# haotianteng/Chiron

Hardware: AMD Instinct MI355X
Metric: kilobases/sec basecalled (DNA_default seg_len=400 batch=1100) (higher is better)
Workload: dtype f32; 1 GPU; DNA_default seg_len=400 jump=390 batch=1100 greedy, synthetic 4 kHz signal (BASELINE.json configs[1]); segment_len=400, jump=390, batch=1100, decode=greedy, weights=seeded synthetic (exact checkpoint shapes), parallelism=reads sharded per GPU, no collective, slots_in_flight=3, parallelism_bookkeeping=none (one rank), distinct_devices=1

## Files before the change

### chiron_amd/csrc/engine.hip

```cpp
#include <hip/hip_runtime.h>

#include <algorithm>
#include <atomic>
#include <chrono>
#include <cfloat>
#include <cmath>
#include <cstdarg>
#include <cstdio>
#include <cstring>
#include <cstdlib>
#include <map>
#include <mutex>
#include <string>
#include <vector>

#include "../../include/chiron_amd.h"
#include "kernels.h"
#include "model_layout.h"
#include "weight_pack.h"
#include <dlfcn.h>

static const char* const kProfNames[] = {"conv_dma", "lstm_proj_dma", "lstm_recurrence", "fc_head", "ctc_greedy", "ctc_beam", "sparse_build",
                                         "path_prob", "conv_lift", "conv_res", "conv1_pwl", "conv_wino", "lstm_proj0_dma", "conv2a"};

// ... 2 lines not shown
static thread_local char g_err[512] = "";
namespace chiron {
chiron_status set_error(chiron_status st, const char* fmt, ...) {
  va_list ap;
  va_start(ap, fmt);
  vsnprintf(g_err, sizeof(g_err), fmt, ap);
  va_end(ap);
  return st;
}
}
static constexpr auto& fail = chiron::set_error;
#define HIP_TRY(expr)                                                                              \
  do {                                                                                             \
    hipError_t _e = (expr);                                                                        \
    if (_e != hipSuccess)                                                                          \
      return fail(CHIRON_ERR_DEVICE, "%s failed: %s (%s:%d)", #expr, hipGetErrorString(_e), __FILE__, \
                  __LINE__);                                                                       \
  } while (0)

extern "C" const char* chiron_last_error(void) { return g_err; }
extern "C" int32_t chiron_abi_version(void) { return CHIRON_ABI_VERSION; }

static int g_timing_build = 0;
static char g_timing_source[96] = "";
namespace chiron {
void mark_timing_build(const char* source) {
  g_timing_build = 1;
  snprintf(g_timing_source, sizeof(g_timing_source), "%s", source ? source : "?");
}
}
extern "C" uint32_t chiron_build_flags(void) { return g_timing_build ? CHIRON_BUILD_TIMING : 0u; }

extern "C" chiron_status chiron_device_pci_bus_id(int32_t device_id, char* out, size_t cap) {
  if (!out || cap < 16) return chiron::set_error(CHIRON_ERR_INVALID, "chiron_device_pci_bus_id: buffer of at least 16 bytes needed");
  int n = 0;
  if (hipGetDeviceCount(&n) != hipSuccess || n <= 0) return chiron::set_error(CHIRON_ERR_DEVICE, "no HIP device");
  if (device_id < 0 || device_id >= n) return chiron::set_error(CHIRON_ERR_INVALID, "device %d of %d", device_id, n);
  hipError_t err = hipDeviceGetPCIBusId(out, (int)cap, device_id);
  if (err != hipSuccess) return chiron::set_error(CHIRON_ERR_DEVICE, "hipDeviceGetPCIBusId: %s", hipGetErrorString(err));
  for (char* c = out; *c; ++c)
    if (*c >= 'A' && *c <= 'F') *c += 'a' - 'A';
  return CHIRON_OK;
}

extern "C" chiron_status chiron_weights_size(const chiron_model_desc* d, size_t* n_floats) {
  BlobMap map;
  chiron_status st = blob_map(d, &map);
  if (st) return st;
  if (!n_floats) return fail(CHIRON_ERR_INVALID, "null n_floats");
  *n_floats = map.total;
  return CHIRON_OK;
}

#define CHIRON_LSTM_WIDE_DEFAULT 2

struct CalibRecord {
  const float* shift;
  int k0, cin;
  int lstm_layer, lstm_dir, lstm_part;
  double rows;
  size_t slot;
};
struct CalibCtx {
  double* dev_sums = nullptr;
  size_t max_records = 0;
  std::vector<CalibRecord> rec;
  int skipped = 0;
};

struct ProfEvent {
  int name_id;
  hipEvent_t a, b;
  double flops, bytes;
};

struct Slot {
  hipStream_t stream = nullptr;
  unsigned long long* tile_ctr = nullptr;
  unsigned long long tile_base = 0;
  unsigned long long tile_base32 = 0;
  float* sig = nullptr;
  int32_t* seq = nullptr;
  float* act[5] = {nullptr, nullptr, nullptr, nullptr, nullptr};
  double* bn_sums = nullptr;
  float* z = nullptr;
  float* lasth[2] = {nullptr, nullptr};
  float* lasth_f32 = nullptr;
  float* logits = nullptr;
  uint8_t* labels = nullptr;
  int32_t* count = nullptr;
  float* log_prob = nullptr;
  float* prob = nullptr;
  int64_t* offsets = nullptr;
  int64_t* indices = nullptr;
  int64_t* values = nullptr;
  int64_t* meta = nullptr;
  void* beam_ws = nullptr;
  size_t beam_ws_bytes = 0;
  float* h_sig = nullptr;
  int32_t* h_seq = nullptr;
  int64_t* h_indices = nullptr;
  int64_t* h_values = nullptr;
  int64_t* h_meta = nullptr;
  float* h_log_prob = nullptr;
  float* h_prob = nullptr;
  float* h_logits = nullptr;
  uint8_t* h_labels = nullptr;
// ... 57 lines not shown
  int calibrated = 0;
  std::vector<void*> owned;
  bool profiling = false;
  std::vector<std::string> prof_names;
  std::mutex mu;
};

static chiron_status dev_alloc(chiron_engine* e, void** p, size_t bytes, bool zero) {
  HIP_TRY(hipMalloc(p, bytes ? bytes : 16));
  e->owned.push_back(*p);
  if (zero) HIP_TRY(hipMemset(*p, 0, bytes ? bytes : 16));
  return CHIRON_OK;
}
static chiron_status upload_plans(chiron_engine* e, std::vector<Upload>& ups) {
  for (Upload& u : ups) {
    chiron_status st = dev_alloc(e, u.dst, u.bytes, false);
    if (st) return st;
    HIP_TRY(hipMemcpy(*u.dst, u.data, u.bytes, hipMemcpyHostToDevice));
    u.owner.reset();
    if (u.host.Npad > 0) e->plan_host[(const float*)*u.dst] = std::move(u.host);
  }
  return CHIRON_OK;
}

static bool split_row_scale() {
  static const bool on = getenv("CHIRON_SPLIT_NO_ROW_SCALE") == nullptr;
  return on;
}

static chiron_status build_plans(chiron_engine* e, const float* w) {
  e->bn_batch = e->desc.bn_mode == CHIRON_BN_BATCH;
  PackSwitches sw;
  sw.no_winograd = getenv("CHIRON_NO_WINOGRAD") != nullptr;
  sw.wino_f2 = getenv("CHIRON_WINOGRAD_F2") != nullptr;
  sw.wino_f4 = getenv("CHIRON_WINOGRAD_F4") != nullptr;
  sw.no_pwl = getenv("CHIRON_NO_PWL") != nullptr;
  sw.split_rec32 = getenv("CHIRON_SPLIT_REC32") != nullptr;
  if (e->split) sw.split_row_scale = split_row_scale();
  std::vector<Upload> ups;
  chiron_status st = pack_weights(e->desc, e->map, w, e->L, e->opts.dtype, sw, e, &ups);
  if (st) return st;
  if (e->proj_bf16 && e->opts.dtype == CHIRON_F32 && !e->bn_batch) {
    for (LstmPlan& lp : e->lstm) {
      ConvGemmPlan& g = lp.proj[0];
      if (lp.nproj != 1 || (lp.in_w != 256 && lp.in_w != 200) || g.N % BF3_BN != 0) continue;
      for (const Upload& u : ups) {
        if (u.dst != reinterpret_cast<void**>(&g.Wt)) continue;
        const std::vector<uint16_t> planes = bf16x3_planes(static_cast<const float*>(u.data), g.N, g.K, lp.in_w);
        if ((st = dev_alloc(e, &g.w_bf3, planes.size() * sizeof(uint16_t), false))) return st;
        HIP_TRY(hipMemcpy(g.w_bf3, planes.data(), planes.size() * sizeof(uint16_t), hipMemcpyHostToDevice));
      }
    }
  }
  return upload_plans(e, ups);
}

static const uint64_t TENSOR_LIMIT = 0xFFFE0000ull;

static chiron_status plan_sizes(const chiron_model_desc* d, const chiron_engine_opts* o, chiron_engine_sizes* out) {
  BlobMap map;
  chiron_status st = blob_map(d, &map);
  if (st) return st;
  if (!o) return fail(CHIRON_ERR_INVALID, "null opts");
  if (o->max_batch < 1 || o->segment_len < 1) return fail(CHIRON_ERR_INVALID, "max_batch/segment_len must be positive");
  if (o->dtype != CHIRON_F32 && o->dtype != CHIRON_F16 && o->dtype != CHIRON_F32_SPLIT && o->dtype != CHIRON_F16_W2)
    return fail(CHIRON_ERR_INVALID, "dtype %d unknown (0 = f32, 1 = f16, 2 = f32 as hi/lo half pairs, 3 = f16 activations against hi/lo weights)", o->dtype);
  if (o->max_beam < 0) return fail(CHIRON_ERR_INVALID, "max_beam %d", o->max_beam);
  const bool f16 = o->dtype == CHIRON_F16 || o->dtype == CHIRON_F16_W2, split = o->dtype == CHIRON_F32_SPLIT, bn_batch = d->bn_mode == CHIRON_BN_BATCH;
  const uint64_t B = (uint64_t)o->max_batch, BP = (uint64_t)roundup(o->max_batch, 16), L = (uint64_t)o->segment_len, H = d->hidden, K = d->classes;
  SiteFrames fr[MAX_SITES];
  const uint64_t T = (uint64_t)frames(map, o->segment_len, fr);
  uint64_t tmax = 0, cmax = 0;
  for (int i = map.has_stem; i < map.n_sites; ++i) {
    tmax = std::max<uint64_t>(tmax, (uint64_t)std::max(fr[i].tin, fr[i].tout));
    cmax = std::max<uint64_t>(cmax, (uint64_t)map.site[i].co);
  }
  const uint64_t lasth_ld = !split ? 2 * H : d->rnn_kind == CHIRON_RNN_MULTI ? 2 * (uint64_t)roundup(d->hidden, 32) : (uint64_t)roundup(2 * d->hidden, 32);
  const uint64_t act = B * tmax * cmax * (f16 ? 2 : 4), lasth = T * BP * lasth_ld * 4, z = T * BP * 2 * 4 * H * 4;
  if (B * tmax >= (1ull << 31) || T * BP >= (1ull << 31))
    return fail(CHIRON_ERR_OVERFLOW, "max_batch %d x %llu frames does not fit the kernels' int row index", o->max_batch, (unsigned long long)tmax);
  if (act > TENSOR_LIMIT)
    return fail(CHIRON_ERR_OVERFLOW, "max_batch %d: an activation tensor [%d x %llu x %llu] needs %llu bytes, the kernels address at most %llu "
                "per tensor (about %llu windows at this segment length and dtype): use a smaller max_batch",
                o->max_batch, o->max_batch, (unsigned long long)tmax, (unsigned long long)cmax, (unsigned long long)act,
                (unsigned long long)TENSOR_LIMIT, (unsigned long long)(TENSOR_LIMIT / (tmax * cmax * (f16 ? 2 : 4))));
  if (T * BP * lasth_ld * (f16 ? 2 : 4) > TENSOR_LIMIT)
    return fail(CHIRON_ERR_OVERFLOW, "max_batch %d: the recurrent output [%llu x %llu x %llu] needs %llu bytes, the kernels address at most %llu per tensor",
                o->max_batch, (unsigned long long)T, (unsigned long long)BP, (unsigned long long)lasth_ld, (unsigned long long)lasth,
                (unsigned long long)TENSOR_LIMIT);
  uint64_t slot = B * L * 4 + BP * 4 + (bn_batch ? 5 : 3) * act + (bn_batch ? 2 * 2 * cmax * 8 : 0) + z + 2 * lasth + (split ? T * BP * 2 * H * 4 : 0);
  slot += B * T * K * 4 + B * T + 3 * B * 4 + (B + 1) * 8 + B * T * 16 + B * T * 8 + 3 * 8;
  if (o->max_beam > 0) slot += beam_workspace_bytes((int)B, (int)T, o->max_beam);
  if (out) {
    out->T = (int32_t)T;
    out->ratio = (double)o->segment_len / (double)T;
    out->largest_tensor_bytes = std::max(act, T * BP * lasth_ld * (f16 ? 2 : 4));
    out->tensor_limit_bytes = TENSOR_LIMIT;
    out->slot_bytes = slot;
    out->total_bytes = slot * (uint64_t)std::max(1, o->n_slots);
  }
  return CHIRON_OK;
}

extern "C" chiron_status chiron_engine_plan(const chiron_model_desc* desc, const chiron_engine_opts* opts, chiron_engine_sizes* out) {
  if (!out) return fail(CHIRON_ERR_INVALID, "null out");
  memset(out, 0, sizeof(*out));
// ... 46 lines not shown
  s->h_flat = (uint8_t*)malloc(B * T ? B * T : 1);
  if (!s->h_flat) return fail(CHIRON_ERR_DEVICE, "out of host memory");
  memset(s->h_prob, 0, B * 4);
  return CHIRON_OK;
}

extern "C" chiron_status chiron_engine_create(const chiron_model_desc* desc, const float* weights, size_t n_floats,
                                              const chiron_engine_opts* opts, chiron_engine** out) {
  if (!out) return fail(CHIRON_ERR_INVALID, "null out");
  *out = nullptr;
  BlobMap map;
  chiron_status st = blob_map(desc, &map);
  if (st) return st;
  if (!weights || !opts) return fail(CHIRON_ERR_INVALID, "null weights/opts");
  if (map.total != n_floats) return fail(CHIRON_ERR_INVALID, "weight blob has %zu floats, descriptor needs %zu", n_floats, map.total);
  {
    chiron_engine_sizes sz;
    if ((st = plan_sizes(desc, opts, &sz))) return st;
  }
  if (desc->hidden != 100) return fail(CHIRON_ERR_INVALID, "hidden=%d: the recurrence kernel is built for hidden=100 (both shipped models)", desc->hidden);
  const bool trace = getenv("CHIRON_TRACE_CREATE") != nullptr;
  auto now = [] { return std::chrono::duration<double, std::milli>(std::chrono::steady_clock::now().time_since_epoch()).count(); };
  const double t_enter = now();
  int ndev = 0;
  if (hipGetDeviceCount(&ndev) != hipSuccess || ndev < 1) return fail(CHIRON_ERR_DEVICE, "no HIP device visible: libchiron_amd has no CPU fallback");
  if (opts->device_id < 0 || opts->device_id >= ndev) return fail(CHIRON_ERR_INVALID, "device_id %d out of range (%d devices)", opts->device_id, ndev);
  HIP_TRY(hipSetDevice(opts->device_id));
  if (trace) HIP_TRY(hipFree(nullptr));
  const double t_runtime = now();

  chiron_engine* e = new chiron_engine();
  e->desc = *desc;
  e->map = map;
  e->opts = *opts;
  if (e->opts.n_slots < 1) e->opts.n_slots = 1;
  e->L = opts->segment_len;
  e->H = desc->hidden;
  e->K = desc->classes;
  e->maxB = opts->max_batch;
  e->BP = roundup(opts->max_batch, 16);
  e->w2 = opts->dtype == CHIRON_F16_W2;
  e->w2_zf16 = e->w2 && getenv("CHIRON_W2_ZF16") != nullptr;
  e->lasth32 = getenv("CHIRON_F16_LASTH16") == nullptr;
  e->f16 = opts->dtype == CHIRON_F16 || e->w2;
  e->split = opts->dtype == CHIRON_F32_SPLIT;
  e->kq = e->f16 ? 2 * GEMM_BK : GEMM_BK;
  e->lasth_ld = !e->split ? 2 * desc->hidden
                : desc->rnn_kind == CHIRON_RNN_MULTI ? 2 * roundup(desc->hidden, 32) : roundup(2 * desc->hidden, 32);
  e->lstm_paired = getenv("CHIRON_LSTM_PAIR") != nullptr;
  e->lstm_fixed_roles = getenv("CHIRON_LSTM_FIXED_ROLES") != nullptr;
  {
    const char* wv = getenv("CHIRON_LSTM_WIDE");
    e->lstm_form = wv ? atoi(wv) : (e->split ? 0 : CHIRON_LSTM_WIDE_DEFAULT);
    if (e->lstm_form < 0 || e->lstm_form > 2) e->lstm_form = CHIRON_LSTM_WIDE_DEFAULT;
  }
  e->lstm16_narrow = getenv("CHIRON_LSTM16_NARROW") != nullptr;
  e->lstm16_pair = getenv("CHIRON_LSTM16_PAIR") ? atoi(getenv("CHIRON_LSTM16_PAIR")) : -1;
  e->stream16 = getenv("CHIRON_NO_STREAM16") == nullptr && opts->dtype != CHIRON_F16_W2;
  e->stream32 = getenv("CHIRON_NO_STREAM32") == nullptr;
  e->proj_bf16 = getenv("CHIRON_PROJ_FP32") == nullptr;
  e->dyn_tiles = getenv("CHIRON_STATIC_TILES") == nullptr;
  {
    const int min_groups = getenv("CHIRON_LSTM16_FUSED_MIN") ? atoi(getenv("CHIRON_LSTM16_FUSED_MIN")) : 64;
    e->lstm16_fused = e->f16 && !e->w2 && !e->lstm16_narrow && desc->hidden == 100 && (e->BP / 16) * 2 >= min_groups && getenv("CHIRON_LSTM16_UNFUSED") == nullptr;
  }
  if (e->f16 && !e->w2) e->host_weights.assign(weights, weights + n_floats);
  st = build_plans(e, weights);
  const double t_plans = now();
  if (st == CHIRON_OK) {
    e->slots.resize(e->opts.n_slots);
    for (Slot& s : e->slots)
      if ((st = alloc_slot(e, &s))) break;
  }
  const double t_slots = now();
  if (st == CHIRON_OK && hipDeviceSynchronize() != hipSuccess) st = fail(CHIRON_ERR_DEVICE, "device sync after setup failed");
  if (trace)
    fprintf(stderr, "chiron_engine_create: {\"hip_runtime_and_context_ms\": %.1f, \"weights_prepared_and_uploaded_ms\": %.1f, \"slot_buffers_ms\": %.1f, "
                    "\"final_sync_ms\": %.1f, \"slots\": %d}\n", t_runtime - t_enter, t_plans - t_runtime, t_slots - t_plans, now() - t_slots, e->opts.n_slots);
  if (st) {
    chiron_engine_destroy(e);
    return st;
  }
  e->prof_names.assign(std::begin(kProfNames), std::end(kProfNames));
  *out = e;
  return CHIRON_OK;
}

extern "C" void chiron_engine_destroy(chiron_engine* e) {
  if (!e) return;
  hipSetDevice(e->opts.device_id);
  hipDeviceSynchronize();
  for (Slot& s : e->slots) {
    for (ProfEvent& ev : s.events) {
      hipEventDestroy(ev.a);
      hipEventDestroy(ev.b);
    }
    if (s.stream) hipStreamDestroy(s.stream);
    void* sp[] = {s.score.labels, s.score.label_len, s.score.loss, s.score.edit, s.score.status, s.score.ws};
    for (void* q : sp)
      if (q) hipFree(q);
    void* hp[] = {s.h_sig, s.h_seq, s.h_indices, s.h_values, s.h_meta, s.h_log_prob, s.h_prob, s.h_logits, s.h_labels, s.h_count};
    free(s.h_flat);
    for (void* q : hp)
      if (q) hipHostFree(q);
  }
  for (void* q : e->owned) hipFree(q);
  delete e;
// ... 272 lines not shown
          Prof pr(e, s, PN_CONV, 2.0 * B * b.t_out * (double)b.k * b.c * b.c, 4.0 * B * (b.t_in + b.t_out) * b.c);
          ok &= launch(e, g, s->stream);
        }
      }
      g = gemm_desc(e, b.gc, B, Mout, b.t_out,
                    {GemmSeg{bufB, b.c, 0, b.c, cop, b.t_out, 1, 0, 0}, GemmSeg{x, b.c_in, 0, b.c_in, cip, b.t_in, b.stride, 0, 0}}, 1, bufA, b.c);
      {
        Prof pr(e, s, PN_CONV, 2.0 * B * b.t_out * (double)(b.c + b.c_in) * b.c, 4.0 * B * b.t_out * (2.0 * b.c + b.c_in));
        ok &= launch(e, g, s->stream);
      }
      x = bufA;
      xi = ia;
    }
  }
  s->sig_used = x;
  return ok;
}

static bool run_rnn(chiron_engine* e, Slot* s, int B) {
  bool ok = true;
  bool last_out_f32 = false;
  const float* fea = s->sig_used;
  const int T = e->T, H = e->H, BP = e->BP;
  const int zc = 4 * H;
  const float* prev = nullptr;
  for (size_t l = 0; l < e->lstm.size(); ++l) {
    const LstmPlan& lp = e->lstm[l];
    float* outbuf = s->lasth[l & 1];
    const bool fused = e->lstm16_fused && lp.wxwide != nullptr;
    for (int pj = 0; pj < (fused ? 0 : lp.nproj); ++pj) {
      const int Kp = roundup(lp.in_w, e->kq);
      const GemmSeg src = l == 0           ? GemmSeg{fea, e->C, 0, e->C, Kp, T, 1, 0, 0}
                          : lp.nproj == 1 ? GemmSeg{prev, e->lasth_ld, 0, 2 * H, Kp, T, 1, 0, 1}
                                          : GemmSeg{prev, e->lasth_ld, e->split ? pj * roundup(H, 32) : pj * H, H, Kp, T, 1, 0, 1};
      GemmParams g = gemm_desc(e, lp.proj[pj], B, (long)T * BP, T, {src}, 0, s->z, 0);
      g.m_time_major = 1;
      g.out_mode = 1;
      g.z_cols = zc;
      g.z_ndir = lp.nproj == 1 ? 2 : 1;
      g.z_dir0 = lp.nproj == 1 ? 0 : pj;
      g.z_seq_len = s->seq;
      g.w_bf3 = lp.proj[pj].w_bf3;
      g.z_f16 = (e->f16 && (!e->w2 || e->w2_zf16)) ? 1 : 0;
      const double ndir = lp.nproj == 1 ? 2.0 : 1.0;
      Prof pr(e, s, l == 0 ? PN_PROJ0 : PN_PROJ, 2.0 * B * T * (double)lp.in_w * 4 * H * ndir, 4.0 * B * T * (lp.in_w + ndir * zc));
      ok &= launch(e, g, s->stream);
    }
    LstmParams r;
    r.z = s->z;
    r.wfrag = lp.wfrag;
    r.wlight = lp.wlight;
    r.wwide = lp.wwide;
    r.wwide32 = lp.wwide32;
    r.wsplit = lp.wsplit;
    r.form32 = e->lstm_form;
    r.narrow16 = e->lstm16_narrow ? 1 : 0;
    r.xsrc = nullptr;
    r.wxwide = nullptr;
    r.whfused = nullptr;
    r.fused_pair = 0;
    r.xbias = nullptr;
    r.xK = r.xld = r.x_time_major = 0;
    if (fused) {
      r.xsrc = l == 0 ? (const void*)fea : (const void*)prev;
      r.wxwide = lp.wxwide;
      r.whfused = lp.whfused;
      r.fused_pair = e->lstm16_pair >= 0 ? (e->lstm16_pair ? 1 : 0) : ((BP / 16) * 2 > current_device_cus() ? 1 : 0);
      r.xbias = lp.proj[0].shift;
      r.xK = lp.in_w;
      r.xld = l == 0 ? e->C : e->lasth_ld;
      r.x_time_major = l == 0 ? 0 : 1;
    }
    r.seq_len = s->seq;
    r.out = e->split ? s->lasth_f32 : outbuf;
    r.out_f32 = (e->f16 && e->lasth32 && e->calib == nullptr && l + 1 == e->lstm.size()) ? 1 : 0;
    last_out_f32 = r.out_f32 != 0;
    const bool direct_split = e->split && lp.wsplit != nullptr && l + 1 < e->lstm.size();
    r.out_split = direct_split ? (void*)outbuf : nullptr;
    r.split_ld = e->lasth_ld;
    r.split_bw0 = e->desc.rnn_kind == CHIRON_RNN_MULTI ? roundup(H, 32) : H;
    r.T = T;
    r.B = B;
    r.BP = BP;
    r.H = H;
    r.ndir = 2;
    r.paired = e->lstm_paired ? 1 : 0;
    r.fixed_roles = e->lstm_fixed_roles ? 1 : 0;
    r.group0 = 0;
    r.f16 = e->f16 ? 1 : 0;
    r.w2 = e->w2 ? (e->w2_zf16 ? 2 : 1) : 0;
    if (e->calib && e->f16) {
      for (int pj = 0; pj < lp.nproj; ++pj) {
        const int dir = lp.nproj == 1 ? -1 : pj;
        if (l == 0)
          calib_measure(e, lp.proj[pj].shift, 0, fea, (long)B * T, e->C, 0, e->C, 0, B, (int)l, dir, 0, s->stream);
        else
          calib_measure(e, lp.proj[pj].shift, 0, prev, (long)T * BP, e->lasth_ld, lp.nproj == 1 ? 0 : pj * H, lp.in_w, BP, B, (int)l, dir, 0, s->stream);
      }
    }
    {
      Prof pr(e, s, PN_REC, 2.0 * 2.0 * B * T * (double)H * 4 * H + (fused ? 2.0 * B * T * (double)lp.in_w * 4 * H * 2.0 : 0.0),
              fused ? (e->f16 ? 2.0 : 4.0) * B * T * (2.0 * lp.in_w + 2.0 * H) : 4.0 * B * T * 2.0 * (zc + H));
      launch_lstm(r, s->stream);
    }
    if (e->calib && e->f16)
      for (int dir = 0; dir < 2; ++dir)
// ... 601 lines not shown
```

### chiron_amd/csrc/kernels.h

```cpp
#pragma once
#include <hip/hip_runtime.h>
#include <stdint.h>

#include "../../include/chiron_amd.h"

#define CHIRON_KMAX 5

namespace chiron {

constexpr int CHIRON_MAX_DEVICES = 64;
inline int current_device_index() {
  int dev = 0;
  if (hipGetDevice(&dev) != hipSuccess || dev < 0 || dev >= CHIRON_MAX_DEVICES) dev = 0;
  return dev;
}
inline int current_device_cus() {
  static int n_cu[CHIRON_MAX_DEVICES] = {};
  const int dev = current_device_index();
  int n = __atomic_load_n(&n_cu[dev], __ATOMIC_RELAXED);
  if (n == 0) {
    hipDeviceProp_t prop;
    n = hipGetDeviceProperties(&prop, dev) == hipSuccess ? prop.multiProcessorCount : 0;
    if (n <= 0) n = 256;
    __atomic_store_n(&n_cu[dev], n, __ATOMIC_RELAXED);
// ... 39 lines not shown
  const float* sig;
  int L;
  const float* lift_a;
  const float* lift_b;
  const float* res_a;
  const float* res_b;
  int res_stride;
  float* out;
  int ldo;
  int out_mode;
  int z_cols;
  int z_ndir;
  int z_dir0;
  int z_dirs_total;
  const int32_t* z_seq_len;
  int f16;
  int z_f16;
  unsigned long long* tile_ctr;
  unsigned long long tile_base;
  unsigned long long* tile_base_host;
};

bool launch_gemm(const GemmParams& p, hipStream_t stream);
bool launch_stream16(const GemmParams& p, hipStream_t stream);
bool launch_stream32(const GemmParams& p, hipStream_t stream);


struct WinoParams {
  const float* src;
  const float* U;
  const float* shift;
  float* out;
  int B, T, C, N, lda, ldo, relu;
  int f4;
  unsigned long long* tile_ctr;
  unsigned long long tile_base;
  unsigned long long* tile_base_host;
};
bool launch_wino_conv3(const WinoParams& p, hipStream_t stream);

constexpr int LSTM_K = 100;
constexpr int LSTM_NW = 7;

struct LstmParams {
  const float* z;
  const float* wfrag;
  const float* wlight;
  const float* wwide32;
  int out_f32;
  const void* wsplit;
  void* out_split;
  int split_ld;
  int split_bw0;
  int form32;
  const void* wwide;
  const void* xsrc;
  const void* wxwide;
  const void* whfused;
  int fused_pair;
  const float* xbias;
  int xK, xld, x_time_major;
  const int32_t* seq_len;
  float* out;
  int T, B, BP, H;
  int ndir;
  int paired;
  int fixed_roles;
  int group0;
  int narrow16;
  int w2;
  int f16;
};
void launch_lstm(const LstmParams& p, hipStream_t stream);
constexpr int LSTM_KSTEPS16 = 25;

void launch_stem_conv(const float* sig, const float* w, const float* shift, void* out, int B, int L, int T_out, int k, int stride, int left,
                      int C, int fmt, int relu, hipStream_t stream);
void launch_split_convert(const float* src, void* dst, long rows, int cols, int ld, int half, int half_dst, hipStream_t stream);
struct PwlConvParams {
  const float* sig;
  const float* bp;
  const float* ref;
  const float2* tab;
  const float* shift;
  void* out;
  int B, L, T_out, k, stride, left, C, nbp;
  int fmt;
};
bool launch_pwl_conv(const PwlConvParams& p, hipStream_t stream);

void launch_lift(const float* sig, const float* a, const float* b, void* out, long n_pos, int C, int fmt ,
                 hipStream_t stream);

struct FcParams {
  const float* lasth;
  const float* w;
  const float* bias;
  const float* wc;
  const float* bc;
  float* logits;
  int T, B, BP, H, K;
  int f16;
  int split;
  int ld;
};
void launch_fc(const FcParams& p, hipStream_t stream);
// ... 169 lines not shown
```

### chiron_amd/csrc/lstm.hip

```cpp
#include "kernels.h"
#include "timing_variants.h"

#include <algorithm>

#pragma clang fp contract(off)

namespace chiron {

typedef float f32x4 __attribute__((ext_vector_type(4)));

constexpr int HG = 8 * 64;

#ifndef CHIRON_GATE_MATH
#define CHIRON_GATE_MATH 0
#endif
typedef float f32x2 __attribute__((ext_vector_type(2)));
constexpr float LOG2E = 1.4426950408889634f;
#if CHIRON_GATE_MATH == 3
__device__ __forceinline__ float sym_tanh(float x) {
  const float e = __builtin_amdgcn_exp2f(__builtin_fabsf(x) * (-2.0f * LOG2E));
  const float t = (1.0f - e) * __builtin_amdgcn_rcpf(1.0f + e);
  return __builtin_copysignf(t, x);
}
#endif
// ... 1303 lines not shown
      if (partial && ch == wave) {
#pragma unroll
        for (int j = 0; j < 8; ++j) {
#pragma unroll
          for (int n = 0; n < 3; ++n) acc[n] = __builtin_amdgcn_mfma_f32_16x16x4f32(w[n][8 * ch + j], hv[ch & 1][j], (ch == 0 && j == 0) ? zero4 : acc[n], 0, 0, 0);
          accp = __builtin_amdgcn_mfma_f32_16x16x4f32(wp[j], hv[ch & 1][j], j == 0 ? zero4 : accp, 0, 0, 0);
        }
      } else {
#pragma unroll
        for (int j = 0; j < 8; ++j)
#pragma unroll
          for (int n = 0; n < 3; ++n) {
#if CHIRON_SENS & 8
            if (j & 1) { acc[n][0] += w[n][8 * ch + j] * hv[ch & 1][j]; continue; }
#endif
            acc[n] = __builtin_amdgcn_mfma_f32_16x16x4f32(w[n][8 * ch + j], hv[ch & 1][j], (ch == 0 && j == 0) ? zero4 : acc[n], 0, 0, 0);
          }
      }
      __builtin_amdgcn_sched_barrier(0);
    }
    __syncthreads();
    const float h24 = hb[(W32_KS - 1) * 64];
#pragma unroll
    for (int n = 0; n < 3; ++n) acc[n] = __builtin_amdgcn_mfma_f32_16x16x4f32(w[n][W32_KS - 1], h24, acc[n], 0, 0, 0);
    f32x4 acc24 = {0.f, 0.f, 0.f, 0.f};
    if (owner24) acc24 = __builtin_amdgcn_mfma_f32_16x16x4f32(wp[0], h24, (f32x4){0.f, 0.f, 0.f, 0.f}, 0, 0, 0);
    asm volatile("s_waitcnt vmcnt(0)" : "+v"(z4[0]), "+v"(z4[1]), "+v"(z4[2]), "+v"(z24) : : "memory");
    if (owner24) reinterpret_cast<f32x4*>(part)[192 + lane] = acc24 + z24;
    if (s > 0) flush(s - 1, cur);
    if (partial) reinterpret_cast<f32x4*>(part)[wave * 64 + lane] = accp;
#pragma unroll
    for (int n = 0; n < 3; ++n) {
      float hnew;
      c[n] = sens_cell(acc[n] + z4[n], c[n], &hnew);
      hbuf[(cur ^ 1) * HW32 + (tile0 + n) * 64 + lane] = hnew;
    }
    cur ^= 1;
    __syncthreads();
  }
  if (maxlen > 0) {
    if (owner24) finish24(cur);
    __syncthreads();
    flush(maxlen - 1, cur);
  }

  for (int s = maxlen; s < p.T; ++s)
    for (int i = tid; i < 16 * p.H; i += 64 * W16_NW) {
      const int r = i / p.H;
      const int uu = i - r * p.H;
      p.out[((long)s * p.BP + g16 * 16 + r) * outw + dir * p.H + uu] = 0.f;
    }
}

static int lstm_cu_count() { return current_device_cus(); }

void launch_lstm(const LstmParams& p0, hipStream_t stream) {
  LstmParams p = p0;
  p.group0 = 0;
  const int groups = p.BP / 4;
  if (p.f16 && p.xsrc) {
    const int g16 = p.BP / 16;
    const dim3 blk(64 * W16_NW);
    if (p.out_f32) {
      static const bool attr_ok = [] {
        return hipFuncSetAttribute(reinterpret_cast<const void*>(lstm16f_kernel<8, 2, true>), hipFuncAttributeMaxDynamicSharedMemorySize, 3 * 2 * 32 * 128 * 2 + 16) == hipSuccess &&
               hipFuncSetAttribute(reinterpret_cast<const void*>(lstm16f_kernel<7, 2, true>), hipFuncAttributeMaxDynamicSharedMemorySize, 3 * 2 * 28 * 128 * 2 + 16) == hipSuccess &&
               hipFuncSetAttribute(reinterpret_cast<const void*>(lstm16f_kernel<8, 1, true>), hipFuncAttributeMaxDynamicSharedMemorySize, 3 * 32 * 128 * 2 + 16) == hipSuccess &&
               hipFuncSetAttribute(reinterpret_cast<const void*>(lstm16f_kernel<7, 1, true>), hipFuncAttributeMaxDynamicSharedMemorySize, 3 * 28 * 128 * 2 + 16) == hipSuccess;
      }();
      (void)attr_ok;
    }
    if (g16 % 2 == 0 && p.fused_pair) {
      const dim3 grd((g16 / 2) * p.ndir);
      if (p.xK > 224) {
        if (p.out_f32) hipLaunchKernelGGL((lstm16f_kernel<8, 2, true>), grd, blk, 3 * 2 * 32 * 128 * 2 + 16, stream, p);
        else hipLaunchKernelGGL((lstm16f_kernel<8, 2>), grd, blk, 3 * 2 * 32 * 128 * 2 + 16, stream, p);
      } else {
        if (p.out_f32) hipLaunchKernelGGL((lstm16f_kernel<7, 2, true>), grd, blk, 3 * 2 * 28 * 128 * 2 + 16, stream, p);
        else hipLaunchKernelGGL((lstm16f_kernel<7, 2>), grd, blk, 3 * 2 * 28 * 128 * 2 + 16, stream, p);
      }
    } else {
      const dim3 grd(g16 * p.ndir);
      if (p.xK > 224) {
        if (p.out_f32) hipLaunchKernelGGL((lstm16f_kernel<8, 1, true>), grd, blk, 3 * 32 * 128 * 2 + 16, stream, p);
        else hipLaunchKernelGGL((lstm16f_kernel<8, 1>), grd, blk, 3 * 32 * 128 * 2 + 16, stream, p);
      } else {
        if (p.out_f32) hipLaunchKernelGGL((lstm16f_kernel<7, 1, true>), grd, blk, 3 * 28 * 128 * 2 + 16, stream, p);
        else hipLaunchKernelGGL((lstm16f_kernel<7, 1>), grd, blk, 3 * 28 * 128 * 2 + 16, stream, p);
      }
    }
    return;
  }
  if (p.f16 && p.w2) {
    if (p.w2 == 2)
      hipLaunchKernelGGL(lstm16w2_kernel<true>, dim3((p.BP / 16) * p.ndir), dim3(64 * W16_NW), 0, stream, p);
    else
      hipLaunchKernelGGL(lstm16w2_kernel<false>, dim3((p.BP / 16) * p.ndir), dim3(64 * W16_NW), 0, stream, p);
    return;
  }
  if (p.f16) {
    const int wide = (p.wwide && !p.narrow16 && (p.BP / 16) * p.ndir >= lstm_cu_count()) ? p.BP / 16 : 0;
    if (wide > 0) hipLaunchKernelGGL(lstm16w_kernel, dim3(wide * p.ndir), dim3(64 * W16_NW), 0, stream, p);
    p.group0 = 4 * wide;
    if (groups > p.group0) hipLaunchKernelGGL(lstm16_kernel, dim3((groups - p.group0) * p.ndir), dim3(64 * LSTM_NW), 0, stream, p);
    return;
  }
  if (p.wsplit) {
    hipLaunchKernelGGL(lstm32s_kernel, dim3((p.BP / 16) * p.ndir), dim3(64 * W16_NW), 0, stream, p);
    return;
  }
  if (p.wwide32 && p.form32 > 0 && !p.paired) {
    if (p.form32 == 2)
      hipLaunchKernelGGL(lstm32w2_kernel, dim3((p.BP / 16) * p.ndir), dim3(64 * W16_NW), 0, stream, p);
    else
      hipLaunchKernelGGL(lstm32w_kernel, dim3((p.BP / 16) * p.ndir), dim3(64 * W16_NW), 0, stream, p);
    return;
  }
  const int n_cu = lstm_cu_count();
  const int pairs = p.paired ? std::min(groups / 2, n_cu / p.ndir) : 0;
  if (pairs > 0) hipLaunchKernelGGL(lstm_kernel<2>, dim3(pairs * p.ndir), dim3(64 * LSTM_NW * 2), 0, stream, p);
  p.group0 = 2 * pairs;
  if (groups > p.group0) hipLaunchKernelGGL(lstm_kernel<1>, dim3((groups - p.group0) * p.ndir), dim3(64 * LSTM_NW), 0, stream, p);
}

}
```

### chiron_amd/csrc/weight_pack.h

```cpp
#pragma once
#include <algorithm>
#include <cfloat>
#include <cmath>
#include <cstdint>
#include <cstring>
#include <memory>
#include <utility>
#include <vector>

#include "kernels.h"
#include "model_layout.h"

namespace chiron {

inline int roundup(int v, int m) { return (v + m - 1) / m * m; }

struct ConvGemmPlan {
  float* Wt = nullptr;
  float* shift = nullptr;
  float* descale = nullptr;
  void* w_bf3 = nullptr;
  int N = 0, Npad = 0, K = 0;
};

struct PlanHost {
  std::vector<float> dW;
  std::vector<float> shift0;
  int N = 0, Npad = 0, K = 0;
};

struct BlockPlan {
  bool lift = false;
  int c_in = 0, c = 0, k = 0, stride = 1, left = 0;
  int t_in = 0, t_out = 0;
  float *lift_a = nullptr, *lift_b = nullptr;
  float *res_a = nullptr, *res_b = nullptr;
  float *pwl_bp = nullptr, *pwl_ref = nullptr, *pwl_tab = nullptr, *pwl_shift = nullptr;
  int pwl_nbp = 0;
  ConvGemmPlan ga, gb, gc;
  float* wino_u = nullptr;
  int wino_f4 = 0;
  ConvGemmPlan g1;
  bool i_bn = false;
  float *bn_scale[4] = {nullptr, nullptr, nullptr, nullptr}, *bn_offset[4] = {nullptr, nullptr, nullptr, nullptr};
};

struct LstmPlan {
  int in_w = 0;
  ConvGemmPlan proj[2];
  int nproj = 1;
  float* wfrag = nullptr;
  void* wwide = nullptr;
  void* whfused = nullptr;
  void* wxwide = nullptr;
  int wx_ksteps = 0;
  void* wsplit = nullptr;
  float* wwide32 = nullptr;
  float* wlight = nullptr;
};

struct NetPlans {
  int T = 0, C = 0;
  int stem_k = 0, stem_stride = 1, stem_left = 0, stem_t = 0, stem_c = 0;
  float *stem_w = nullptr, *stem_shift = nullptr, *stem_scale = nullptr, *stem_offset = nullptr;
  std::vector<BlockPlan> blocks;
  std::vector<LstmPlan> lstm;
  float *fc_w = nullptr, *fc_b = nullptr, *fc_wc = nullptr, *fc_bc = nullptr;
};

struct PackSwitches {
  bool no_winograd = false;
  bool wino_f2 = false;
  bool wino_f4 = false;
  bool no_pwl = false;
  bool split_rec32 = false;
  bool split_row_scale = true;
};

struct Upload {
  void** dst;
  std::shared_ptr<void> owner;
  const void* data;
  size_t bytes;
  PlanHost host;
};


struct HalfPair {
  _Float16 hi, lo;
};
inline HalfPair split_half(float v) {
  const _Float16 hi = (_Float16)v;
  return {hi, (_Float16)(v - (float)hi)};
}

struct Bf16x3 {
  uint16_t hi, mid, lo;
};
inline uint32_t f32_bits(float v) {
  uint32_t u;
  memcpy(&u, &v, 4);
  return u;
}
inline float bits_f32(uint32_t u) {
  float v;
  memcpy(&v, &u, 4);
  return v;
}
inline Bf16x3 split_bf16x3(float w) {
  const uint32_t hb = f32_bits(w) & 0xffff0000u;
// ... 33 lines not shown
    const float inv = (1.0f / sqrtf(var[i] + 1e-5f)) * scale[i];
    f.inv[i] = inv;
    f.sh[i] = offset[i] - mean[i] * inv;
  }
  return f;
}

inline void fold_filter(std::vector<float>& Wt, std::vector<float>& shift, int K, int k0, const float* W, int taps, int ci, int co, int cop,
                        const float* inv, const float* sh) {
  for (int n = 0; n < co; ++n) {
    for (int tap = 0; tap < taps; ++tap)
      for (int c = 0; c < ci; ++c) {
        const float v = W[((size_t)tap * ci + c) * co + n];
        Wt[(size_t)n * K + k0 + tap * cop + c] = inv ? v * inv[n] : v;
      }
    if (sh) shift[n] = k0 == 0 ? sh[n] : shift[n] + sh[n];
  }
}

struct LstmKernels {
  const float* kern[2];
  int H;
  float at(int dir, int k_off, int width, int k, int g, int unit) const {
    return k < width && unit < H ? kern[dir][(size_t)(k_off + k) * 4 * H + g * H + unit] : 0.f;
  }
};

template <class Put>
inline void narrow_fragments(const LstmKernels& kn, int V, int ksteps, int k_off, int width, Put put) {
  for (int dir = 0; dir < 2; ++dir)
    for (int wv = 0; wv < LSTM_NW; ++wv)
      for (int ks = 0; ks < ksteps; ++ks)
        for (int lane = 0; lane < 64; ++lane)
          for (int q = 0; q < V; ++q) {
            const int k = V * ks + q, g = lane >> 4, unit = 16 * wv + (lane & 15);
            put(((((size_t)dir * LSTM_NW + wv) * ksteps + ks) * 64 + lane) * V + q, kn.at(dir, k_off, width, k, g, unit));
          }
}
inline size_t narrow_elems(int V, int ksteps) { return (size_t)2 * LSTM_NW * ksteps * 64 * V; }

template <class Put>
inline void wide_fragments(const LstmKernels& kn, int V, int ksteps, int k_off, int width, Put put) {
  for (int dir = 0; dir < 2; ++dir)
    for (int wv = 0; wv < 8; ++wv)
      for (int slot = 0; slot < (wv == 7 ? 4 : 3); ++slot)
        for (int ks = 0; ks < ksteps; ++ks)
          for (int lane = 0; lane < 64; ++lane)
            for (int q = 0; q < V; ++q) {
              const int k = V * (4 * ks + (lane >> 4)) + q, g = lane & 3, unit = 4 * (3 * wv + slot) + ((lane >> 2) & 3);
              put((((((size_t)dir * 8 + wv) * 4 + slot) * ksteps + ks) * 64 + lane) * V + q, kn.at(dir, k_off, width, k, g, unit));
            }
}
inline size_t wide_elems(int V, int ksteps) { return (size_t)2 * 8 * 4 * ksteps * 64 * V; }

inline std::vector<float> light_fragment(const LstmKernels& kn, int k_off) {
  std::vector<float> wl((size_t)2 * 28 * 64, 0.f);
  for (int dir = 0; dir < 2; ++dir)
    for (int m = 0; m < 28; ++m)
      for (int lane = 0; lane < 64; ++lane) {
        const int q = m >> 2, a = m & 3, kg = lane >> 4, g = (lane >> 2) & 3, j = lane & 3;
        const int k = 16 * q + 4 * kg + a;
        wl[((size_t)dir * 28 + m) * 64 + lane] = kn.at(dir, k_off, kn.H, k, g, 96 + j);
      }
  return wl;
}

struct WeightPacker {
  const chiron_model_desc& d;
  const BlobMap& map;
  const float* w;
  const PackSwitches sw;
  const bool f16, w2, split, batch;
  const int kq;
  NetPlans* out;
  std::vector<Upload>* ups;

  template <class P, class Tp>
  Upload& put(P** dst, std::vector<Tp>&& h) {
    auto v = std::make_shared<std::vector<Tp>>(std::move(h));
    ups->push_back(Upload{reinterpret_cast<void**>(dst), v, v->data(), v->size() * sizeof(Tp), PlanHost()});
    return ups->back();
  }

  void gemm(ConvGemmPlan* g, std::vector<float>&& Wt, std::vector<float>&& shift, int N, int Npad, int K) {
    g->N = N;
    g->Npad = Npad;
    g->K = K;
    if (split) {
      std::vector<_Float16> h(2 * Wt.size());
      std::vector<float> sh2(std::move(shift)), ds((size_t)Npad + 192, 1.0f);
      for (int n = 0; n < Npad; ++n) {
        float mx = 0.f;
        for (int k = 0; k < K; ++k) mx = std::max(mx, fabsf(Wt[(size_t)n * K + k]));
        int s = 0;
        if (sw.split_row_scale && mx > 0.f && std::isfinite(mx)) {
          int ex;
          frexpf(mx, &ex);
          s = std::min(60, std::max(-60, 13 - ex));
          if (n < (int)sh2.size() && !std::isfinite(ldexpf(sh2[n], s))) s = 0;
        }
        ds[n] = ldexpf(1.0f, -s);
        if (n < (int)sh2.size()) sh2[n] = ldexpf(sh2[n], s);
        for (int k = 0; k < K; ++k) {
          const size_t i = (size_t)n * K + k;
          const HalfPair p = split_half(ldexpf(Wt[i], s));
          const size_t blk = i / 32, el = i % 32;
// ... 295 lines not shown
```

Measured before the change: 5010 kbases/s.

## Run f32 LSTM recurrence as bf16x3 split MFMA by default

Adds a new LSTM recurrence kernel (form 3, now the default) that splits the recurrent weights and hidden state into three bf16 planes each. The first 96 of the K dimension is accumulated with nine 16x16x32 bf16 MFMA cross terms, and the remaining slice uses an f32 MFMA. The hidden state is re-split into bf16 planes in LDS at every step. The aim is to replace slow f32 4-wide MFMA work in the serial recurrence with denser bf16 MFMA while keeping near-f32 accuracy, at the cost of more MFMA instructions, more registers and extra LDS traffic.

```diff
diff --git a/chiron_amd/csrc/engine.hip b/chiron_amd/csrc/engine.hip
--- a/chiron_amd/csrc/engine.hip
+++ b/chiron_amd/csrc/engine.hip
@@ -78,7 +78,7 @@
   return CHIRON_OK;
 }
 
-#define CHIRON_LSTM_WIDE_DEFAULT 2
+#define CHIRON_LSTM_WIDE_DEFAULT 3
 
 struct CalibRecord {
   const float* shift;
@@ -242,6 +242,13 @@
       }
     }
   }
+  for (LstmPlan& lp : e->lstm)
+    for (const Upload& u : ups) {
+      if (u.dst != reinterpret_cast<void**>(&lp.wwide32)) continue;
+      const std::vector<uint16_t> frag = rec_bf16x3_fragments(static_cast<const float*>(u.data));
+      if ((st = dev_alloc(e, &lp.wrec_bf3, frag.size() * sizeof(uint16_t), false))) return st;
+      HIP_TRY(hipMemcpy(lp.wrec_bf3, frag.data(), frag.size() * sizeof(uint16_t), hipMemcpyHostToDevice));
+    }
   return upload_plans(e, ups);
 }
 
@@ -394,7 +401,7 @@
   {
     const char* wv = getenv("CHIRON_LSTM_WIDE");
     e->lstm_form = wv ? atoi(wv) : (e->split ? 0 : CHIRON_LSTM_WIDE_DEFAULT);
-    if (e->lstm_form < 0 || e->lstm_form > 2) e->lstm_form = CHIRON_LSTM_WIDE_DEFAULT;
+    if (e->lstm_form < 0 || e->lstm_form > 3) e->lstm_form = CHIRON_LSTM_WIDE_DEFAULT;
   }
   e->lstm16_narrow = getenv("CHIRON_LSTM16_NARROW") != nullptr;
   e->lstm16_pair = getenv("CHIRON_LSTM16_PAIR") ? atoi(getenv("CHIRON_LSTM16_PAIR")) : -1;
@@ -773,6 +780,7 @@
     r.wlight = lp.wlight;
     r.wwide = lp.wwide;
     r.wwide32 = lp.wwide32;
+    r.wrec_bf3 = lp.wrec_bf3;
     r.wsplit = lp.wsplit;
     r.form32 = e->lstm_form;
     r.narrow16 = e->lstm16_narrow ? 1 : 0;
diff --git a/chiron_amd/csrc/kernels.h b/chiron_amd/csrc/kernels.h
--- a/chiron_amd/csrc/kernels.h
+++ b/chiron_amd/csrc/kernels.h
@@ -115,6 +115,7 @@
   void* out_split;
   int split_ld;
   int split_bw0;
+  const void* wrec_bf3;
   int form32;
   const void* wwide;
   const void* xsrc;
diff --git a/chiron_amd/csrc/lstm.hip b/chiron_amd/csrc/lstm.hip
--- a/chiron_amd/csrc/lstm.hip
+++ b/chiron_amd/csrc/lstm.hip
@@ -1379,6 +1379,187 @@
     }
 }
 
+typedef __bf16 bf16x8 __attribute__((ext_vector_type(8)));
+constexpr int REC_BF3_TERMS = 9;
+constexpr bool REC_BF3_SMALL_FIRST = true;
+constexpr bool REC_BF3_LEAN = false;
+constexpr int HPL = 3 * 3 * 64;
+
+template <bool LEAN>
+__global__ __launch_bounds__(64 * W16_NW, 1) void lstm32w2_kernel_bf3(const LstmParams p) {
+  __shared__ __attribute__((aligned(16))) float hbuf[2 * HW32];
+  __shared__ __attribute__((aligned(16))) float part[4 * 256];
+  __shared__ __attribute__((aligned(16))) f32x4 hpl[2 * HPL];
+  __shared__ __attribute__((aligned(16))) f32x4 wp_lds[LEAN ? 3 * 3 * 64 : 1];
+
+  const int tid = threadIdx.x;
+  const int lane = tid & 63;
+  const int wave = __builtin_amdgcn_readfirstlane(tid >> 6);
+  const int dir = blockIdx.x % p.ndir;
+  const int g16 = blockIdx.x / p.ndir;
+  const int tile0 = 3 * wave;
+  const bool partial = wave < 3, owner24 = wave == W16_NW - 1;
+  const f32x4 zero4 = {0.f, 0.f, 0.f, 0.f};
+
+  bf16x8 wb[3][3][3], wpb[3];
+  float wl[3], wp0 = 0.f;
+  {
+    const f32x4* wrec = reinterpret_cast<const f32x4*>(p.wrec_bf3) + (long)dir * 25 * 9 * 64 + lane;
+#pragma unroll
+    for (int n = 0; n < 3; ++n)
+#pragma unroll
+      for (int j = 0; j < 9; ++j) wb[n][j / 3][j % 3] = __builtin_bit_cast(bf16x8, wrec[((tile0 + n) * 9 + j) * 64]);
+    const float* wf = p.wwide32 + ((long)dir * W16_NW + wave) * W16_NT * W32_KS * 64 + lane;
+#pragma unroll
+    for (int n = 0; n < 3; ++n) wl[n] = wf[(n * W32_KS + W32_KS - 1) * 64];
+    if (owner24) wp0 = p.wwide32[((((long)dir * W16_NW + 7) * W16_NT + 3) * W32_KS + W32_KS - 1) * 64 + lane];
+#pragma unroll
+    for (int pl = 0; pl < 3; ++pl) {
+      f32x4 v = zero4;
+      if (partial) v = wrec[((24 * 3 + wave) * 3 + pl) * 64];
+      if (LEAN) {
+        if (partial) wp_lds[(wave * 3 + pl) * 64 + lane] = v;
+      } else {
+        wpb[pl] = __builtin_bit_cast(bf16x8, v);
+      }
+    }
+  }
+  for (int i = tid; i < 2 * HW32; i += 64 * W16_NW) hbuf[i] = 0.f;
+  for (int i = tid; i < 2 * HPL; i += 64 * W16_NW) hpl[i] = zero4;
+
+  const int row = lane & 15, q = lane >> 4;
+  int maxlen = 0;
+#pragma unroll
+  for (int r = 0; r < 16; ++r) maxlen = max(maxlen, min(p.seq_len[g16 * 16 + r], p.T));
+  __syncthreads();
+
+  const unsigned outw = p.ndir * p.H;
+  const unsigned zcols = 4 * p.H;
+  const unsigned zstep = (p.BP >> 2) * p.ndir * zcols * 4;
+  const unsigned zlo = (((((g16 * 4 + (row >> 2)) * p.ndir + dir) * zcols + 4 * tile0 + q) * 4) + (row & 3)) * 4;
+  const unsigned zhi = zlo + 2 * 1600;
+  const unsigned ostep = p.BP * outw;
+  const int hpw = row * 8 + q;
+
+  const int f_len = min(p.seq_len[g16 * 16 + (lane & 15)], p.T);
+  auto flush = [&](int sp, int buf) {
+    int lo = lane;
+    asm volatile("" : "+v"(lo));
+    const int fr = lo & 15, fq = 4 * wave + (lo >> 4);
+    if (fq < 25) {
+      const bool act = sp < f_len;
+      const unsigned to = (dir == 0 || !act) ? sp : f_len - 1 - sp;
+      const float* hp = hbuf + buf * HW32 + fq * 64 + fr;
+      f32x4 v = {hp[0], hp[16], hp[32], hp[48]};
+      if (!act) v = zero4;
+      *reinterpret_cast<f32x4*>(p.out + (to * ostep + (g16 * 16 + fr) * outw + dir * p.H + 4 * fq)) = v;
+    }
+  };
+
+  float c[3] = {0.f, 0.f, 0.f};
+  float c24 = 0.f;
+  int cur = 0;
+
+  auto finish24 = [&](int buf) {
+    const f32x4* pp = reinterpret_cast<const f32x4*>(part) + lane;
+    f32x4 sum = pp[0] + pp[64];
+    sum = sum + pp[128];
+    float hnew;
+    c24 = sens_cell(sum + pp[192], c24, &hnew);
+    hbuf[buf * HW32 + 24 * 64 + lane] = hnew;
+  };
+
+  constexpr int TERMS[9][2] = {{2, 2}, {2, 1}, {1, 2}, {2, 0}, {1, 1}, {0, 2}, {1, 0}, {0, 1}, {0, 0}};
+  constexpr int T0 = 9 - REC_BF3_TERMS;
+
+  for (int s = 0; s < maxlen; ++s) {
+    const float* zs = p.z + (size_t)s * zstep;
+    f32x4 z4[3], z24 = zero4;
+    W32_ZLOAD(z4[0][0], zlo, 0);   W32_ZLOAD(z4[0][1], zlo, 1600);   W32_ZLOAD(z4[0][2], zhi, 0);   W32_ZLOAD(z4[0][3], zhi, 1600);
+    W32_ZLOAD(z4[1][0], zlo, 64);  W32_ZLOAD(z4[1][1], zlo, 1664);   W32_ZLOAD(z4[1][2], zhi, 64);  W32_ZLOAD(z4[1][3], zhi, 1664);
+    W32_ZLOAD(z4[2][0], zlo, 128); W32_ZLOAD(z4[2][1], zlo, 1728);   W32_ZLOAD(z4[2][2], zhi, 128); W32_ZLOAD(z4[2][3], zhi, 1728);
+    if (owner24) {
+      W32_ZLOAD(z24[0], zlo, 192); W32_ZLOAD(z24[1], zlo, 1792); W32_ZLOAD(z24[2], zhi, 192); W32_ZLOAD(z24[3], zhi, 1792);
+    }
+    if (owner24 && s > 0) finish24(cur);
+    const f32x4* hp = hpl + cur * HPL + lane;
+    f32x4 acc[3], accp = zero4;
+    bf16x8 hb[LEAN ? 2 : 3][3];
+#pragma unroll
+    for (int j = 0; j < (LEAN ? 3 : 9); ++j) hb[LEAN ? 0 : j % 3][j / (LEAN ? 1 : 3)] = __builtin_bit_cast(bf16x8, hp[(LEAN ? 3 * j : j) * 64]);
+#pragma unroll
+    for (int ks = 0; ks < 3; ++ks) {
+      if (LEAN && ks < 2) {
+#pragma unroll
+        for (int pl = 0; pl < 3; ++pl) hb[(ks + 1) & 1][pl] = __builtin_bit_cast(bf16x8, hp[(pl * 3 + ks + 1) * 64]);
+      }
+      const bf16x8* hk = hb[LEAN ? ks & 1 : ks];
+      if (partial && ks == wave) {
+        bf16x8 wq[3];
+#pragma unroll
+        for (int pl = 0; pl < 3; ++pl) wq[pl] = LEAN ? __builtin_bit_cast(bf16x8, wp_lds[(ks * 3 + pl) * 64 + lane]) : wpb[pl];
+#pragma unroll
+        for (int i = 0; i < REC_BF3_TERMS; ++i) {
+          const int t = REC_BF3_SMALL_FIRST ? i + T0 : 8 - i;
+#pragma unroll
+          for (int n = 0; n < 3; ++n)
+            acc[n] = __builtin_amdgcn_mfma_f32_16x16x32_bf16(wb[n][ks][TERMS[t][0]], hk[TERMS[t][1]], (ks == 0 && i == 0) ? zero4 : acc[n], 0, 0, 0);
+          accp = __builtin_amdgcn_mfma_f32_16x16x32_bf16(wq[TERMS[t][0]], hk[TERMS[t][1]], i == 0 ? zero4 : accp, 0, 0, 0);
+        }
+      } else {
+#pragma unroll
+        for (int i = 0; i < REC_BF3_TERMS; ++i) {
+          const int t = REC_BF3_SMALL_FIRST ? i + T0 : 8 - i;
+#pragma unroll
+          for (int n = 0; n < 3; ++n)
+            acc[n] = __builtin_amdgcn_mfma_f32_16x16x32_bf16(wb[n][ks][TERMS[t][0]], hk[TERMS[t][1]], (ks == 0 && i == 0) ? zero4 : acc[n], 0, 0, 0);
+        }
+      }
+      __builtin_amdgcn_sched_barrier(0);
+    }
+    __syncthreads();
+    const float h24 = hbuf[cur * HW32 + (W32_KS - 1) * 64 + lane];
+#pragma unroll
+    for (int n = 0; n < 3; ++n) acc[n] = __builtin_amdgcn_mfma_f32_16x16x4f32(wl[n], h24, acc[n], 0, 0, 0);
+    f32x4 acc24 = zero4;
+    if (owner24) acc24 = __builtin_amdgcn_mfma_f32_16x16x4f32(wp0, h24, zero4, 0, 0, 0);
+    asm volatile("s_waitcnt vmcnt(0)" : "+v"(z4[0]), "+v"(z4[1]), "+v"(z4[2]), "+v"(z24) : : "memory");
+    if (owner24) reinterpret_cast<f32x4*>(part)[192 + lane] = acc24 + z24;
+    if (s > 0) flush(s - 1, cur);
+    if (partial) reinterpret_cast<f32x4*>(part)[wave * 64 + lane] = accp;
+    unsigned short* const hq = reinterpret_cast<unsigned short*>(hpl + (cur ^ 1) * HPL) + hpw;
+#pragma unroll
+    for (int n = 0; n < 3; ++n) {
+      float hnew;
+      c[n] = sens_cell(acc[n] + z4[n], c[n], &hnew);
+      hbuf[(cur ^ 1) * HW32 + (tile0 + n) * 64 + lane] = hnew;
+      const int tl = tile0 + n;
+      const int at = ((tl >> 3) * 64 + ((tl & 7) >> 1) * 16) * 8 + 4 * (tl & 1);
+      const unsigned xb = __builtin_bit_cast(unsigned, hnew);
+      const float r = hnew - __builtin_bit_cast(float, xb & 0xffff0000u);
+      const unsigned rb = __builtin_bit_cast(unsigned, r);
+      const float lo = r - __builtin_bit_cast(float, rb & 0xffff0000u);
+      hq[at] = (unsigned short)(xb >> 16);
+      hq[at + 3 * 512] = (unsigned short)(rb >> 16);
+      hq[at + 6 * 512] = (unsigned short)(__builtin_bit_cast(unsigned, lo) >> 16);
+    }
+    cur ^= 1;
+    __syncthreads();
+  }
+  if (maxlen > 0) {
+    if (owner24) finish24(cur);
+    __syncthreads();
+    flush(maxlen - 1, cur);
+  }
+
+  for (int s = maxlen; s < p.T; ++s)
+    for (int i = tid; i < 16 * p.H; i += 64 * W16_NW) {
+      const int r = i / p.H;
+      const int uu = i - r * p.H;
+      p.out[((long)s * p.BP + g16 * 16 + r) * outw + dir * p.H + uu] = 0.f;
+    }
+}
+
 static int lstm_cu_count() { return current_device_cus(); }
 
 void launch_lstm(const LstmParams& p0, hipStream_t stream) {
@@ -1437,7 +1618,9 @@
     return;
   }
   if (p.wwide32 && p.form32 > 0 && !p.paired) {
-    if (p.form32 == 2)
+    if (p.form32 == 3)
+      hipLaunchKernelGGL(lstm32w2_kernel_bf3<REC_BF3_LEAN>, dim3((p.BP / 16) * p.ndir), dim3(64 * W16_NW), 0, stream, p);
+    else if (p.form32 == 2)
       hipLaunchKernelGGL(lstm32w2_kernel, dim3((p.BP / 16) * p.ndir), dim3(64 * W16_NW), 0, stream, p);
     else
       hipLaunchKernelGGL(lstm32w_kernel, dim3((p.BP / 16) * p.ndir), dim3(64 * W16_NW), 0, stream, p);
diff --git a/chiron_amd/csrc/weight_pack.h b/chiron_amd/csrc/weight_pack.h
--- a/chiron_amd/csrc/weight_pack.h
+++ b/chiron_amd/csrc/weight_pack.h
@@ -56,6 +56,7 @@
   int wx_ksteps = 0;
   void* wsplit = nullptr;
   float* wwide32 = nullptr;
+  void* wrec_bf3 = nullptr;
   float* wlight = nullptr;
 };
 
@@ -195,6 +196,31 @@
             }
 }
 inline size_t wide_elems(int V, int ksteps) { return (size_t)2 * 8 * 4 * ksteps * 64 * V; }
+
+inline size_t wide32_index(int dir, int k, int gate, int unit) {
+  const int tile = unit >> 2, wv = tile == 24 ? 7 : tile / 3, slot = tile - 3 * wv;
+  return (((((size_t)dir * 8 + wv) * 4 + slot) * 25 + (k >> 2)) * 64) + (size_t)((k & 3) * 16 + 4 * (unit & 3) + gate);
+}
+
+constexpr int REC_BF3_K = 96;
+inline size_t rec_bf16x3_index(int dir, int plane, int k, int gate, int unit) {
+  const int tile = unit >> 2, ks = k >> 5, lane = ((k >> 3) & 3) * 16 + 4 * (unit & 3) + gate;
+  return (((((size_t)dir * 25 + tile) * 3 + ks) * 3 + plane) * 64 + lane) * 8 + (size_t)(k & 7);
+}
+inline size_t rec_bf16x3_elems() { return (size_t)2 * 25 * 3 * 3 * 64 * 8; }
+inline std::vector<uint16_t> rec_bf16x3_fragments(const float* ww) {
+  std::vector<uint16_t> v(rec_bf16x3_elems(), (uint16_t)0);
+  for (int dir = 0; dir < 2; ++dir)
+    for (int unit = 0; unit < 100; ++unit)
+      for (int gate = 0; gate < 4; ++gate)
+        for (int k = 0; k < REC_BF3_K; ++k) {
+          const Bf16x3 s = split_bf16x3(ww[wide32_index(dir, k, gate, unit)]);
+          v[rec_bf16x3_index(dir, 0, k, gate, unit)] = s.hi;
+          v[rec_bf16x3_index(dir, 1, k, gate, unit)] = s.mid;
+          v[rec_bf16x3_index(dir, 2, k, gate, unit)] = s.lo;
+        }
+  return v;
+}
 
 inline std::vector<float> light_fragment(const LstmKernels& kn, int k_off) {
   std::vector<float> wl((size_t)2 * 28 * 64, 0.f);
```

Result: no change. 4998 kbases/s, median of 4 (-0.2%).
